# evalf/nutils

Hardware: AMD Instinct MI355X
Metric: elements assembled/sec (global stiffness K) (higher is better)
Workload: dtype f64; 1 GPU; 3D Poisson stiffness, 128^3 structured hex, p=1, 2x2x2 Gauss, iso geometry (BASELINE.json configs[1]); nelems_per_gpu=2097152, nnz_per_gpu=57066625, kernel=k_p1hex_skew<16,16,false,false>, parallelism=single GPU, launch=hipGraph replay (20 steps per graph), settle_steps=600

## Files before the change

nutils_amd/csrc/nh_assemble_p1hex.hip:

```cpp
#include "nh_common.h"
#include <algorithm>
#include <type_traits>
#include <cstdio>
#include <cstdlib>

namespace {

#ifdef NH_ABLATION
#define DEBUG(p) ((p).debug)
#else
#define DEBUG(p) 0
#endif

struct P1Args {
  int n0, n1, n2;
  int lay0, lay1;
  int pl0, pl1;
  const double *verts;
  double origin[3], scale[3];
  double n[2][2];
  double c[3][2];
  double wk[2][2][2];
  double wm[2][2][2];
  int hasm;
// ... 268 lines not shown
          if (kact && (flag & need) == need) {
            const bool below = !upper && dI < 0;
            const double *src0 = acc + (below ? slot_of(Pb - 1) : slot_of(Pb)) + srow, *src1 = acc + (below ? slot_of(Pb) : slot_of(Pb + 1)) + srow;
            double v0[OJ], v1[OJ];
#pragma unroll
            for (int oj = 0; oj < OJ; ++oj) v0[oj] = src0[oj * (VK * NS)];
#pragma unroll
            for (int oj = 0; oj < OJ; ++oj) v1[oj] = src1[oj * (VK * NS)];
            char *lp0 = reinterpret_cast<char *>(p.values + ((3 * (i64)Pb - 1) * T1 * T2 + 3 * (cumJ0 * T2)));
            char *lp1 = lp0 + 8 * (3 * T1 * T2);
#pragma unroll
            for (int oj = 0; oj < OJ; ++oj) {
              *reinterpret_cast<double *>(lp0 + voff8) = v0[oj];
              lp0 += stride8;
            }
#pragma unroll
            for (int oj = 0; oj < OJ; ++oj) {
              *reinterpret_cast<double *>(lp1 + voff8) = v1[oj];
              lp1 += stride8;
            }
          }
        } else if (!lowJ && !highJ) planes(std::integral_constant<int, 0>{});
        else if (!(lowJ && highJ)) planes(std::integral_constant<int, 1>{});
        else planes(std::integral_constant<int, 2>{});
      }
    }
    NH_TICK(4)
    if (last) break;
    lds_barrier();
    NH_TICK(5)
    if (fresh) {
      for (int t = tid; t < NP * PS / 2; t += NT) reinterpret_cast<double2 *>(acc)[t] = make_double2(0., 0.);
    } else {
#pragma unroll
      for (int P = L0 - 1; P < L0 + L - 1; ++P) {
        double2 *z = reinterpret_cast<double2 *>(acc + slot_of(P));
        for (int t = tid; t < PS / 2; t += NT) z[t] = make_double2(0., 0.);
      }
    }
    col = ncol, A = nA, B = nB, L0 = nL0;
    NH_TICK(6)
  }
#ifdef NH_ABLATION
  if (p.tdbg && (tid & 63) == 0)
    for (int i = 0; i < 8; ++i) atomicAdd((unsigned long long *)p.tdbg + i, (unsigned long long)tacc[i]);
#endif
}
#undef NH_TICK

__device__ __forceinline__ void half_arrive(unsigned *cnt) {
  asm volatile("s_waitcnt lgkmcnt(0)" ::: "memory");
  if ((threadIdx.x & 63) == 0) atomicAdd(cnt, 1u);
}
__device__ __forceinline__ void half_wait(unsigned *cnt, unsigned target) {
  while (__hip_atomic_load(cnt, __ATOMIC_RELAXED, __HIP_MEMORY_SCOPE_WORKGROUP) < target) __builtin_amdgcn_s_sleep(1);
  asm volatile("" ::: "memory");
}

#ifdef NH_P1HEX_WPE
#define NH_WPE __attribute__((amdgpu_waves_per_eu(2, 2)))
#else
#define NH_WPE
#endif
template <int TJ, int TK, bool MASS, bool COEF>
__global__ __launch_bounds__(2 * TJ * TK) NH_WPE void k_p1hex_skew(P1Args p) {
  constexpr bool VEC = false;
#ifdef NH_ABLATION
  long long tacc[10] = {0, 0, 0, 0, 0, 0, 0, 0, 0, 0}, tprev = clock64();
  const long long tstart = tprev;
  int nslow = 0, nfast = 0;
#ifdef NH_NOTICKS
#define NH_TICK(i)
#else
#define NH_TICK(i) { const long long tnow = clock64(); tacc[i] += tnow - tprev; tprev = tnow; }
#endif
#else
#define NH_TICK(i)
#endif
  constexpr int G = TJ * TK, NT = 2 * G, NP = 4, OJ = TJ - 1, OK = TK - 1, NS = 15, VW = 3;
  constexpr int VJ = TJ + 1, VK = TK + 1, RP = VJ * VK, PS = (RP * NS + 1) & ~1, VPG = (RP + G - 1) / G;
  const bool getenv_stage_late = p.wbnd < 0;
  extern __shared__ __attribute__((aligned(16))) double lds[];
  double *acc = lds;
  double *vbuf = lds + NP * PS;
  unsigned *hcnt = reinterpret_cast<unsigned *>(vbuf + 3 * RP * VW);
  const int tid = threadIdx.x, lt = tid & (G - 1), grp = __builtin_amdgcn_readfirstlane(tid / G);
  const int N0 = p.n0 + 1, N1 = p.n1 + 1, N2 = p.n2 + 1;
  const int NPL = p.pl1 - p.pl0;
  const unsigned wg = gridDim.x % 8 == 0 ? (blockIdx.x % 8) * (gridDim.x / 8) + blockIdx.x / 8 : blockIdx.x;
  const i64 CP = NPL + 2, WI = 16, WB = p.nbj > 1 ? (p.wbnd < 0 ? -p.wbnd : p.wbnd) : 16;
  const i64 rowB = p.nbk * CP * WB, rowI = p.nbk * CP * WI, nmid = max(p.nbj - 2, 0);
  const i64 ctot = (p.nbj > 1 ? 2 : 1) * rowB + nmid * rowI;
  auto unit_at = [&](i64 c) {
    i64 jt, rem, w;
    if (c < rowB) jt = 0, rem = c, w = WB;
    else if (c < rowB + nmid * rowI) jt = 1 + (c - rowB) / rowI, rem = (c - rowB) % rowI, w = WI;
    else jt = p.nbj > 1 ? p.nbj - 1 : 1, rem = c - rowB - nmid * rowI, w = WB;
    const i64 kt = rem / (CP * w), pos = (rem - kt * CP * w) / w;
    return (jt * p.nbk + kt) * NPL + min(max(pos - 1, (i64)0), (i64)NPL);
  };
  i64 u = unit_at(ctot * wg / gridDim.x);
  const i64 u1 = unit_at(ctot * (wg + 1) / gridDim.x);
  if (u >= u1) return;
  auto slot_of = [](int P) { return (int)((unsigned)(P + 2 * NP) % NP) * PS; };
  auto vslot_of = [](int P) { return (int)((unsigned)(P + 3) % 3) * (RP * VW); };
  auto load_vertex = [&](int I, int r, int J0, int K0, double (&x)[3]) {
    const int bb = r / VK, c = r % VK, J = J0 - 1 + bb, K = K0 - 1 + c;
    x[0] = x[1] = x[2] = 0.;
    if (r < RP && I >= 0 && I < N0 && J >= 0 && J < N1 && K >= 0 && K < N2) {
      const double *src = p.verts + (((i64)I * N1 + J) * N2 + K) * 3;
      x[0] = src[0], x[1] = src[1], x[2] = src[2];
    }
  };
  if (tid == 0) *hcnt = 0;
  unsigned htarget = 0;
  const i64 T1 = 3 * (i64)N1 - 2, T2 = 3 * (i64)N2 - 2;
  while (u < u1) {
    const int col = (int)(u / NPL), A = p.pl0 + (int)(u % NPL), B = (int)min((i64)p.pl1, A + (u1 - u));
    const int J0 = (col / p.nbk) * OJ, K0 = (col % p.nbk) * OK;
    {
      constexpr int NVL = (2 * RP + NT - 1) / NT;
      double x[NVL][3];
      bool valid[NVL];
#pragma unroll
      for (int k = 0; k < NVL; ++k) {
        const int v = min(tid + k * NT, 2 * RP - 1), pl = v / RP, r = v % RP, I = A - 1 + pl;
        const int J = J0 - 1 + r / VK, K = K0 - 1 + r % VK;
        valid[k] = I >= 0 && I < N0 && J >= 0 && J < N1 && K >= 0 && K < N2;
        const double *src = p.verts + (((i64)min(max(I, 0), N0 - 1) * N1 + min(max(J, 0), N1 - 1)) * N2 + min(max(K, 0), N2 - 1)) * 3;
        x[k][0] = src[0], x[k][1] = src[1], x[k][2] = src[2];
      }
      for (int t = tid; t < NP * PS / 2; t += NT) reinterpret_cast<double2 *>(acc)[t] = make_double2(0., 0.);
#pragma unroll
      for (int k = 0; k < NVL; ++k) {
        const int v = tid + k * NT, pl = v / RP, r = v % RP;
        if (v < 2 * RP) {
          double *dst = vbuf + vslot_of(A - 1 + pl) + r * VW;
          dst[0] = valid[k] ? x[k][0] : 0., dst[1] = valid[k] ? x[k][1] : 0., dst[2] = valid[k] ? x[k][2] : 0.;
        }
      }
    }
    lds_barrier();

    for (int s = A - 1; s <= B; ++s) {
      htarget += G / 64;
      NH_TICK(0)
      const bool mathrole = ((s - (A - 1)) & 1) == grp;
#ifdef NH_P1HEX_PRIO
      if (mathrole == (NH_P1HEX_PRIO == 1)) __builtin_amdgcn_s_setprio(3); else __builtin_amdgcn_s_setprio(0);
#endif
      if (mathrole) {
        const int ej = lt / TK, ek = lt % TK;
        const int gi = s, gj = J0 - 1 + ej, gk = K0 - 1 + ek;
        if (s < B && gi >= p.lay0 && gi < p.lay1 && gj >= 0 && gj < p.n1 && gk >= 0 && gk < p.n2 && !(DEBUG(p) & 4)) {
#define NH_P1HEX_VERT(a, bb, c) (vbuf + vslot_of(gi + (a)) + ((ej + (bb)) * VK + (ek + (c))) * VW)
#include "nh_p1hex_element.inc"
#undef NH_P1HEX_VERT
        }
        NH_TICK(3)
      } else {
        const bool needv = s + 1 < B && !(DEBUG(p) & 8);
        double Vn[VPG][3];
#pragma unroll
        for (int k = 0; k < VPG; ++k) load_vertex(needv ? s + 2 : -1, lt + k * G, J0, K0, Vn[k]);
        const int P = s - 1;
        bool arrived = false, staged = false, recycled = false;
        auto stage_vertices = [&]() {
#pragma unroll
          for (int k = 0; k < VPG; ++k) {
            const int r = lt + k * G;
            if (r < RP) {
              double *dst = vbuf + vslot_of(s + 2) + r * VW;
              dst[0] = Vn[k][0], dst[1] = Vn[k][1], dst[2] = Vn[k][2];
            }
          }
        };
        if (P >= A && !(DEBUG(p) & 2)) {
          const bool lowJ = J0 == 0, highJ = J0 + OJ >= N1;
          const int cumJ0 = J0 == 0 ? 0 : 3 * J0 - 1;
#ifdef NH_ABLATION
          if (!lowJ && !highJ && P > 0 && P < N0 - 1 && K0 > 0 && K0 + OK < N2) ++nfast; else ++nslow;
#endif
          if (!lowJ && !highJ && P > 0 && P < N0 - 1 && K0 > 0 && K0 + OK < N2) {
            const int e = 2 * lt;
            auto source = [&](int ee, bool &below) {
              const int ok_ = ee / 27, sl_ = ee - ok_ * 27;
              const int dJ_ = (sl_ / 3) % 3 - 1, dK_ = sl_ % 3 - 1;
              below = sl_ < 9;
              return (VK + ok_ + 1) * NS + (sl_ >= 13 ? sl_ - 13 : (dJ_ * VK + dK_) * NS + 13 - sl_);
            };
#ifdef NH_P1HEX_PIPEFLUSH
            constexpr int D = NH_P1HEX_PIPEFLUSH;
            const int ec = 2 * min(lt, 201);
            bool belowA, belowB;
            const int offA = source(ec, belowA), offB = source(ec + 1, belowB);
            const double *sA = acc + (belowA ? slot_of(P - 1) : slot_of(P)) + offA;
            const double *sB = acc + (belowB ? slot_of(P - 1) : slot_of(P)) + offB;
            const int li = lt - 202;
            const bool lone = li >= 0 && li < OJ;
            bool belowL;
            const int offL = source(404, belowL);
            const double aL = acc[(belowL ? slot_of(P - 1) : slot_of(P)) + offL + (lone ? li : 0) * (VK * NS)];
            const i64 stride8 = 8 * (i64)(9 * (int)T2);
            char *l0 = reinterpret_cast<char *>(p.values + ((3 * (i64)P - 1) * T1 * T2 + 3 * (cumJ0 * T2) + 9 * (3 * (i64)K0 - 1)));
            char *lp = l0 + 8 * ec;
            double a0[OJ], a1[OJ];
#pragma unroll
            for (int i = 0; i < D && i < OJ; ++i) a0[i] = sA[i * (VK * NS)], a1[i] = sB[i * (VK * NS)];
            __builtin_amdgcn_sched_barrier(0);
#pragma unroll
            for (int i = 0; i < OJ; ++i) {
              if (i + D < OJ) a0[i + D] = sA[(i + D) * (VK * NS)], a1[i + D] = sB[(i + D) * (VK * NS)];
              __builtin_amdgcn_sched_barrier(0);
              const double2 v = make_double2(a0[i], a1[i]);
              __builtin_memcpy(lp + i * stride8, &v, 16);
              __builtin_amdgcn_sched_barrier(0);
            }
            half_arrive(hcnt);
            arrived = true;
            if (needv) {
              stage_vertices();
              staged = true;
            }
            __builtin_amdgcn_sched_barrier(0);
            if (lone) *reinterpret_cast<double *>(l0 + li * stride8 + 8 * 404) = aL;
#else
            bool belowA, belowB;
            const int offA = source(e < 405 ? e : 404, belowA), offB = source(e + 1 < 405 ? e + 1 : 404, belowB);
            const double *sA = acc + (belowA ? slot_of(P - 1) : slot_of(P)) + offA;
            const double *sB = acc + (belowB ? slot_of(P - 1) : slot_of(P)) + offB;
            double a0[OJ], a1[OJ];
#pragma unroll
            for (int i = 0; i < OJ; ++i) {
              a0[i] = sA[i * (VK * NS)];
              a1[i] = sB[i * (VK * NS)];
            }
            const int li = lt - 202;
            const bool lone = li >= 0 && li < OJ;
            bool belowL;
            const int offL = source(404, belowL);
            const double aL = acc[(belowL ? slot_of(P - 1) : slot_of(P)) + offL + (lone ? li : 0) * (VK * NS)];
            half_arrive(hcnt);
            arrived = true;
            NH_TICK(8)
            if (needv && !getenv_stage_late) {
              __builtin_amdgcn_s_waitcnt(0x0f70);
              stage_vertices();
              staged = true;
            }
            const i64 stride8 = 8 * (i64)(9 * (int)T2);
            char *l0 = reinterpret_cast<char *>(p.values + ((3 * (i64)P - 1) * T1 * T2 + 3 * (cumJ0 * T2) + 9 * (3 * (i64)K0 - 1)));
            char *lp = l0 + 16 * lt;
#ifdef NH_P1HEX_INTERLEAVE
            half_wait(hcnt, htarget);
            recycled = true;
            {
              double2 *z = reinterpret_cast<double2 *>(acc + slot_of(s - 2));
              constexpr int NZ = (PS / 2 + G - 1) / G;
              static_assert(NZ <= OJ, "one zeroing write per store");
#pragma unroll
              for (int i = 0; i < OJ; ++i) {
                if (lt < 202) {
                  const double2 v = make_double2(a0[i], a1[i]);
                  __builtin_memcpy(lp + i * stride8, &v, 16);
                }
                if (i < NZ && lt + i * G < PS / 2) z[lt + i * G] = make_double2(0., 0.);
                __builtin_amdgcn_sched_barrier(0);
              }
            }
#else
            if (lt < 202) {
#pragma unroll
              for (int i = 0; i < OJ; ++i) {
                if ((DEBUG(p) & 16) && (i & 1)) continue;
                const double2 v = make_double2(a0[i], a1[i]);
                __builtin_memcpy(lp + i * stride8, &v, 16);
              }
            }
#endif
            if (lone) *reinterpret_cast<double *>(l0 + li * stride8 + 8 * 404) = aL;
#endif
          } else {
            constexpr int RPP = G / 32, KP = (OK + RPP - 1) / RPP;
            const int sl = lt & 31, rsub = lt >> 5;
            const int dI = sl / 9 - 1, dJ = (sl / 3) % 3 - 1, dK = sl % 3 - 1;
            const bool upper = sl >= 13;
            const int need = (dI < 0 ? 1 : dI > 0 ? 8 : 0) | (dJ < 0 ? 2 : dJ > 0 ? 16 : 0) | (dK < 0 ? 4 : dK > 0 ? 32 : 0);
            const int loI = P > 0, hiI = P < N0 - 1, lenI = loI + 1 + hiI;
            double v[KP][OJ];
#pragma unroll
            for (int kp = 0; kp < KP; ++kp) {
              const int ok = kp * RPP + rsub;
              const int srow = (VK + ok + 1) * NS + (upper ? sl - 13 : (dJ * VK + dK) * NS + 13 - sl);
              const double *src = acc + ((!upper && dI < 0) ? slot_of(P - 1) : slot_of(P)) + (ok < OK ? srow : 0);
#pragma unroll
              for (int oj = 0; oj < OJ; ++oj) v[kp][oj] = src[oj * (VK * NS)];
            }
            half_arrive(hcnt);
            arrived = true;
#pragma unroll
            for (int kp = 0; kp < KP; ++kp) {
              const int ok = kp * RPP + rsub, Kk = K0 + ok;
              const bool kact = sl < 27 && ok < OK && Kk < N2;
              const int loK = Kk > 0, hiK = Kk < N2 - 1, lenK = loK + 1 + hiK, cumK = Kk == 0 ? 0 : 3 * Kk - 1;
              double *line = p.values + ((P == 0 ? 0 : 3 * (i64)P - 1) * T1 * T2 + lenI * (cumJ0 * T2));
              if (!lowJ && !highJ) {
                const int flag = loI | 2 | loK << 2 | hiI << 3 | 16 | hiK << 5;
                const unsigned voff8 = 8u * (unsigned)(lenI * 3 * cumK + ((dI + loI) * 3 + (dJ + 1)) * lenK + (dK + loK));
                const i64 stride8 = 8 * (i64)(lenI * 3 * (int)T2);
                if (kact && (flag & need) == need) {
                  char *lp = reinterpret_cast<char *>(line);
#pragma unroll
                  for (int oj = 0; oj < OJ; ++oj) {
                    if (!((DEBUG(p) & 16) && (oj & 1))) *reinterpret_cast<double *>(lp + voff8) = v[kp][oj];
                    lp += stride8;
                  }
                }
              } else {
#pragma unroll
                for (int oj = 0; oj < OJ; ++oj) {
                  const int J = J0 + oj;
                  const int loJ = J > 0, hiJ = J < N1 - 1, lenJ = loJ + 1 + hiJ;
                  const int flag = loI | loJ << 1 | loK << 2 | hiI << 3 | hiJ << 4 | hiK << 5;
                  const unsigned voff = (unsigned)(lenI * lenJ * cumK + ((dI + loI) * lenJ + (dJ + loJ)) * lenK + (dK + loK));
                  if (kact && J < N1 && (flag & need) == need && !((DEBUG(p) & 16) && (oj & 1))) line[voff] = v[kp][oj];
                  line += lenI * lenJ * (int)T2;
                }
              }
            }
          }
        }
        NH_TICK(6)
        if (!arrived) half_arrive(hcnt);
        if (!recycled) half_wait(hcnt, htarget);
        NH_TICK(7)
        if (!recycled) {
          double2 *z = reinterpret_cast<double2 *>(acc + slot_of(s - 2));
          for (int t = lt; t < PS / 2; t += G) z[t] = make_double2(0., 0.);
        }
        NH_TICK(9)
        if (needv && !staged) stage_vertices();
      }
      if (mathrole) { NH_TICK(1) } else { NH_TICK(4) }
      lds_barrier();
      if (mathrole) { NH_TICK(2) } else { NH_TICK(5) }
    }
    u += B - A;
  }
#ifdef NH_ABLATION
  if (p.tdbg && tid == 0) {
    p.tdbg[16 + 4 * blockIdx.x] = clock64() - tstart;
    p.tdbg[16 + 4 * blockIdx.x + 1] = nfast;
    p.tdbg[16 + 4 * blockIdx.x + 2] = nslow;
  }
  if (p.tdbg && (tid & 63) == 0)
    for (int i = 0; i < 10; ++i) atomicAdd((unsigned long long *)p.tdbg + i, (unsigned long long)tacc[i]);
#endif
}
#undef NH_TICK

#include "nh_p1hex_tiles.inc"
#include "nh_p1hex_tri.inc"

__global__ void k_p1hex_unit_matrix(P1Args p, double *Ke) {
  double X[2][2][2][3];
  for (int a = 0; a < 2; ++a)
    for (int b = 0; b < 2; ++b)
      for (int c = 0; c < 2; ++c) {
        X[a][b][c][0] = p.origin[0] + p.scale[0] * a;
        X[a][b][c][1] = p.origin[1] + p.scale[1] * b;
        X[a][b][c][2] = p.origin[2] + p.scale[2] * c;
      }
  ElemTables T;
  {
    double (&R0)[3][3] = T.R0, (&R1)[3][3] = T.R1, (&R2)[3][3] = T.R2;
    double (&W01)[2][2][3] = T.W01, (&W02)[2][2][3] = T.W02, (&W12)[2][2][3] = T.W12;
    double (&Mm)[3][3][3] = T.Mm;
    for (int i = 0; i < 27; ++i) (&Mm[0][0][0])[i] = 0.;
    const bool hasm = p.hasm;
#define NH_P1HEX_QS(q) 1.
#define NH_P1HEX_QM(q) 1.
#include "nh_p1hex_math.inc"
#undef NH_P1HEX_QS
#undef NH_P1HEX_QM
  }
#pragma unroll
  for (int a = 0; a < 8; ++a)
#pragma unroll
    for (int b = 0; b < 8; ++b) Ke[a * 8 + b] = element_entry(T, a < b ? a : b, a < b ? b : a);
}

__global__ __launch_bounds__(256) void k_p1hex_uniform(P1Args p, const double *KeG) {
  __shared__ double Ke[64], tabI[2 * 27], tabF[18], tabL[18];
  if (threadIdx.x < 64) Ke[threadIdx.x] = KeG[threadIdx.x];
  __syncthreads();
  const int N0 = p.n0 + 1, N1 = p.n1 + 1, N2 = p.n2 + 1;
  const int I = p.pl0 + blockIdx.x / N1, J = blockIdx.x % N1;
  const i64 T1 = 3 * (i64)N1 - 2, T2 = 3 * (i64)N2 - 2;
// ... 61 lines not shown
  const int slot = (int)(t % 27);
  if (row > row1 || (row == row1 && slot != 0)) return;
  const i64 T1 = 3 * (i64)N1 - 2, T2 = 3 * (i64)N2 - 2;
  auto rp = [&](i64 r) -> i64 {
    if (r >= (i64)N0 * N1 * N2) return (3 * (i64)N0 - 2) * T1 * T2;
    const int Kk = (int)(r % N2), J = (int)((r / N2) % N1), I = (int)(r / ((i64)N2 * N1));
    return cum_of(I, N0) * T1 * T2 + len_of(I, N0) * (cum_of(J, N1) * T2 + (i64)len_of(J, N1) * cum_of(Kk, N2));
  };
  const i64 base = rp(row0);
  if (slot == 0) rowptr[row - row0] = rp(row) - base;
  if (row >= row1) return;
  const int Kk = (int)(row % N2), J = (int)((row / N2) % N1), I = (int)(row / ((i64)N2 * N1));
  const int dI = slot / 9 - 1, dJ = (slot / 3) % 3 - 1, dK = slot % 3 - 1;
  const int cI = I + dI, cJ = J + dJ, cK = Kk + dK;
  if (cI < 0 || cI >= N0 || cJ < 0 || cJ >= N1 || cK < 0 || cK >= N2) return;
  const int lenJ = len_of(J, N1), lenK = len_of(Kk, N2);
  const int pos = ((dI + (I > 0)) * lenJ + (dJ + (J > 0))) * lenK + (dK + (Kk > 0));
  colidx[rp(row) - base + pos] = ((i64)cI * N1 + cJ) * N2 + cK;
}

}

template <bool VEC, bool MASS, bool COEF>
static int launch_march_inst(const nh_p1hex_args *a, P1Args &p, void *stream) {
#ifdef NH_ABLATION
  p.debug = getenv("NH_P1HEX_DEBUG") ? atoi(getenv("NH_P1HEX_DEBUG")) : 0;
#endif
  static const int wbnd_env = getenv("NH_P1HEX_WBND") ? std::min(64, std::max(8, atoi(getenv("NH_P1HEX_WBND")))) : 20;
  p.wbnd = getenv("NH_P1HEX_STAGE_LATE") ? -wbnd_env : wbnd_env;
  constexpr int TJ = 16, TK = 16, L = 2, NTM = L * TJ * TK, NS = VEC ? 1 : 15, VW = VEC ? 4 : 3;
  int dev = 0;
  NH_CHECK_HIP(hipGetDevice(&dev));
  NH_REQUIRE(dev >= 0 && dev < 16, "nh_p1hex: device index %d not supported", dev);
  static int cus_of[16] = {0};
  if (!cus_of[dev]) {
    int n = 256;
    NH_CHECK_HIP(hipDeviceGetAttribute(&n, hipDeviceAttributeMultiprocessorCount, dev));
    cus_of[dev] = n;
  }
  const int cus = cus_of[dev];
  p.nbj = (p.n1 + 1 + TJ - 2) / (TJ - 1);
  p.nbk = (p.n2 + 1 + TK - 2) / (TK - 1);
  const size_t ldsm = sizeof(double) * ((L + 2) * (((TJ + 1) * (TK + 1) * NS + 1) & ~1) + (L + 1) * (TJ + 1) * (TK + 1) * VW + 2);
  const i64 units = (i64)p.nbj * p.nbk * (p.pl1 - p.pl0);
  NH_REQUIRE(a->max_workgroups >= 0, "nh_p1hex: negative max_workgroups");
  unsigned grid = (unsigned)std::min<i64>(units, a->max_workgroups ? std::min(cus, a->max_workgroups) : cus);
#ifdef NH_ABLATION
  if (getenv("NH_P1HEX_MAXWG")) grid = std::min<unsigned>(grid, (unsigned)atoi(getenv("NH_P1HEX_MAXWG")));
#endif
  auto kern = k_p1hex_march<TJ, TK, L, VEC, MASS, COEF>;
  if constexpr (!VEC && L == 2) {
    const char *env = getenv("NH_P1HEX_MARCH"), *kenv = getenv("NH_P1HEX_KERNEL");
    const bool march = (env && atoi(env)) || (kenv && !strcmp(kenv, "march"));
    if (!march) kern = k_p1hex_skew<TJ, TK, MASS, COEF>;
  }
  static const void *attr_set[16][2] = {{nullptr, nullptr}};
  if (attr_set[dev][0] != (const void *)kern && attr_set[dev][1] != (const void *)kern) {
    NH_CHECK_HIP(hipFuncSetAttribute((const void *)kern, hipFuncAttributeMaxDynamicSharedMemorySize, (int)ldsm));
    attr_set[dev][attr_set[dev][0] ? 1 : 0] = (const void *)kern;
  }
#ifdef NH_ABLATION
  static long long *tdbg = nullptr;
  if (!tdbg) NH_CHECK_HIP(hipMalloc((void **)&tdbg, (16 + 4 * 1024) * sizeof(long long)));
  NH_CHECK_HIP(hipMemsetAsync(tdbg, 0, (16 + 4 * 1024) * sizeof(long long), nh_stream(stream)));
  p.tdbg = getenv("NH_P1HEX_TIMERS") ? tdbg : nullptr;
#endif
  hipLaunchKernelGGL(kern, dim3(grid), dim3(NTM), ldsm, nh_stream(stream), p);
  NH_LAUNCH_CHECK();
#ifdef NH_ABLATION
  if (p.tdbg) {
    static long long h[16 + 4 * 1024];
    NH_CHECK_HIP(hipMemcpy(h, tdbg, sizeof h, hipMemcpyDeviceToHost));
    if (getenv("NH_P1HEX_WGTIMES"))
      for (unsigned g = 0; g < grid; ++g) fprintf(stderr, "wg %u cycles %lld fast %lld slow %lld\n", g, h[16 + 4 * g], h[16 + 4 * g + 1], h[16 + 4 * g + 2]);
    const double nw = (double)grid * (NTM / 64);
    if (kern != (void (*)(P1Args))k_p1hex_march<TJ, TK, L, VEC, MASS, COEF>)
      fprintf(stderr, "p1hex_skew cycles per wave: prologue %.0f | math %.0f | - %.0f | math wait %.0f | lds reads %.0f | store issue %.0f | half wait %.0f | zero %.0f | stage %.0f | mem wait %.0f\n", h[0] / nw, h[3] / nw, h[1] / nw,
              h[2] / nw, h[8] / nw, h[6] / nw, h[7] / nw, h[9] / nw, h[4] / nw, h[5] / nw);
    else
    fprintf(stderr, "p1hex_march cycles per wave: stage+next %.0f | B1 %.0f | load+math %.0f | B2 %.0f | stage+flush %.0f | B3 %.0f | zero %.0f\n", h[0] / nw, h[1] / nw,
            h[2] / nw, h[3] / nw, h[4] / nw, h[5] / nw, h[6] / nw);
  }
#endif
  return NH_OK;
}


namespace {
struct TileScratch {
  void *base = nullptr;
  size_t cap = 0;
  unsigned *err_host = nullptr, *err_dev = nullptr;
};
TileScratch g_tiles[16];
}

int nh_p1hex_tiles_release(void) {
  for (auto &t : g_tiles) {
    if (t.base) NH_CHECK_HIP(hipFree(t.base));
    t.base = nullptr, t.cap = 0;
  }
  return NH_OK;
}

template <bool MASS, bool COEF>
static int launch_tiles_inst(const nh_p1hex_args *a, P1Args &p, void *stream) {
  using namespace p1t;
// ... 252 lines not shown
```

nutils_amd/csrc/nh_p1hex_apply.inc:

```
{
  const double (&n)[2][2] = p.n;
  double J0[2][2][3], J1[2][2][3], J2[2][2][3], g0[2][2], g1[2][2], g2[2][2];
#pragma unroll
  for (int d = 0; d < 4; ++d) {
    double e0[2][2], e1[2][2], e2[2][2];
#pragma unroll
    for (int x = 0; x < 2; ++x)
#pragma unroll
      for (int y = 0; y < 2; ++y) {
        if (d < 3) {
          e0[x][y] = X[1][x][y][d < 3 ? d : 0] - X[0][x][y][d < 3 ? d : 0];
          e1[x][y] = X[x][1][y][d < 3 ? d : 0] - X[x][0][y][d < 3 ? d : 0];
          e2[x][y] = X[x][y][1][d < 3 ? d : 0] - X[x][y][0][d < 3 ? d : 0];
        } else {
          e0[x][y] = un[4 + x * 2 + y] - un[x * 2 + y];
          e1[x][y] = un[x * 4 + 2 + y] - un[x * 4 + y];
          e2[x][y] = un[x * 4 + y * 2 + 1] - un[x * 4 + y * 2];
        }
      }
#pragma unroll
    for (int q1 = 0; q1 < 2; ++q1) {
      double t0[2], t1[2], t2[2];
#pragma unroll
      for (int y = 0; y < 2; ++y) {
        t0[y] = n[0][q1] * e0[0][y] + n[1][q1] * e0[1][y];
        t1[y] = n[0][q1] * e1[0][y] + n[1][q1] * e1[1][y];
        t2[y] = n[0][q1] * e2[0][y] + n[1][q1] * e2[1][y];
      }
#pragma unroll
      for (int q2 = 0; q2 < 2; ++q2) {
        const double v0 = n[0][q2] * t0[0] + n[1][q2] * t0[1], v1 = n[0][q2] * t1[0] + n[1][q2] * t1[1], v2 = n[0][q2] * t2[0] + n[1][q2] * t2[1];
        if (d < 3) {
          J0[q1][q2][d < 3 ? d : 0] = v0;
          J1[q1][q2][d < 3 ? d : 0] = v1;
          J2[q1][q2][d < 3 ? d : 0] = v2;
        } else {
          g0[q1][q2] = v0;
          g1[q1][q2] = v1;
          g2[q1][q2] = v2;
        }
      }
    }
  }
  double uq[2][2][2];
  if (hasm) {
    double ua[2][2][2], ub[2][2][2];
#pragma unroll
    for (int x = 0; x < 2; ++x)
#pragma unroll
      for (int y = 0; y < 2; ++y)
#pragma unroll
        for (int qc = 0; qc < 2; ++qc) ua[x][y][qc] = n[0][qc] * un[x * 4 + y * 2] + n[1][qc] * un[x * 4 + y * 2 + 1];
#pragma unroll
    for (int x = 0; x < 2; ++x)
// ... 98 lines not shown
```

nutils_amd/csrc/nh_p1hex_math.inc:

```
{
  const double (&n)[2][2] = p.n;
  const double (&c)[3][2] = p.c;
  double J0[2][2][3], J1[2][2][3], J2[2][2][3];
#pragma unroll
  for (int d = 0; d < 3; ++d) {
    double e0[2][2], e1[2][2], e2[2][2];
#pragma unroll
    for (int x = 0; x < 2; ++x)
#pragma unroll
      for (int y = 0; y < 2; ++y) {
        e0[x][y] = X[1][x][y][d] - X[0][x][y][d];
        e1[x][y] = X[x][1][y][d] - X[x][0][y][d];
        e2[x][y] = X[x][y][1][d] - X[x][y][0][d];
      }
    double t0[2][2], t1[2][2], t2[2][2];
#pragma unroll
    for (int y = 0; y < 2; ++y) {
      const double d0 = e0[1][y] - e0[0][y], d1 = e1[1][y] - e1[0][y], d2 = e2[1][y] - e2[0][y];
#pragma unroll
      for (int q1 = 0; q1 < 2; ++q1) {
        t0[q1][y] = fma(n[1][q1], d0, e0[0][y]);
        t1[q1][y] = fma(n[1][q1], d1, e1[0][y]);
        t2[q1][y] = fma(n[1][q1], d2, e2[0][y]);
      }
    }
#pragma unroll
    for (int q1 = 0; q1 < 2; ++q1) {
      const double d0 = t0[q1][1] - t0[q1][0], d1 = t1[q1][1] - t1[q1][0], d2 = t2[q1][1] - t2[q1][0];
#pragma unroll
      for (int q2 = 0; q2 < 2; ++q2) {
        J0[q1][q2][d] = fma(n[1][q2], d0, t0[q1][0]);
        J1[q1][q2][d] = fma(n[1][q2], d1, t1[q1][0]);
        J2[q1][q2][d] = fma(n[1][q2], d2, t2[q1][0]);
      }
    }
  }
  double D0[2][2], D1[2][2], D2[2][2], M01[2][2][2], M02[2][2][2], M12[2][2][2], Dm[2][2][2];
#pragma unroll
  for (int qa = 0; qa < 2; ++qa)
#pragma unroll
    for (int qb = 0; qb < 2; ++qb)
#pragma unroll
      for (int qc = 0; qc < 2; ++qc) {
        const double *c0 = J0[qb][qc], *c1 = J1[qa][qc], *c2 = J2[qa][qb];
        double A[3][3];
        A[0][0] = c1[1] * c2[2] - c1[2] * c2[1];
        A[0][1] = c1[2] * c2[0] - c1[0] * c2[2];
        A[0][2] = c1[0] * c2[1] - c1[1] * c2[0];
        A[1][0] = c2[1] * c0[2] - c2[2] * c0[1];
        A[1][1] = c2[2] * c0[0] - c2[0] * c0[2];
        A[1][2] = c2[0] * c0[1] - c2[1] * c0[0];
        A[2][0] = c0[1] * c1[2] - c0[2] * c1[1];
        A[2][1] = c0[2] * c1[0] - c0[0] * c1[2];
        A[2][2] = c0[0] * c1[1] - c0[1] * c1[0];
        const double det = c0[0] * A[0][0] + c0[1] * A[0][1] + c0[2] * A[0][2];
// ... 130 lines not shown
```

Baseline: 12.29 billion elements/s.

## Cut address arithmetic and register pressure in skewed p1hex assembly kernel

Reworks the skewed-wavefront hex assembly loop to carry rotating ring indices, vertex slot offsets and the global output line pointer incrementally instead of recomputing modulo and 64-bit index math each plane. The state moves to 32-bit unsigned scheduling values made uniform via readfirstlane, and kernel arguments are read through a scalar kernarg pointer. Per-lane LDS source offsets are hoisted out of the loop, and the scatter reads use inline-asm ds_read_b64 with immediate offsets. Other changes: a single-lane wave arrive via exec masking, a boundary-lane mask hoisted per column, and unrolled slot zeroing. It adds a host-side limit check for 32-bit overflow and removes the pipeflush/interleave variants.

Measured after the change: 12.25 billion elements/s. About the same (-0.3%).

```diff
diff --git a/nutils_amd/csrc/nh_assemble_p1hex.hip b/nutils_amd/csrc/nh_assemble_p1hex.hip
--- a/nutils_amd/csrc/nh_assemble_p1hex.hip
+++ b/nutils_amd/csrc/nh_assemble_p1hex.hip
@@ -344,6 +344,11 @@
   asm volatile("s_waitcnt lgkmcnt(0)" ::: "memory");
   if ((threadIdx.x & 63) == 0) atomicAdd(cnt, 1u);
 }
+__device__ __forceinline__ void half_arrive_wave(unsigned *cnt) {
+  unsigned long long saved;
+  asm volatile("s_waitcnt lgkmcnt(0)\n\ts_mov_b64 %0, exec\n\ts_mov_b64 exec, 1\n\tds_add_u32 %1, %2\n\ts_mov_b64 exec, %0"
+               : "=&s"(saved) : "v"((unsigned)(size_t)cnt), "v"(1u) : "memory");
+}
 __device__ __forceinline__ void half_wait(unsigned *cnt, unsigned target) {
   while (__hip_atomic_load(cnt, __ATOMIC_RELAXED, __HIP_MEMORY_SCOPE_WORKGROUP) < target) __builtin_amdgcn_s_sleep(1);
   asm volatile("" ::: "memory");
@@ -354,6 +359,32 @@
 #else
 #define NH_WPE
 #endif
+__device__ __forceinline__ int uni(int x) { return __builtin_amdgcn_readfirstlane(x); }
+__device__ __forceinline__ unsigned lane_offset(unsigned x) {
+  asm volatile("" : "+v"(x));
+  return x;
+}
+typedef double double2v __attribute__((ext_vector_type(2)));
+template <int OFF>
+__device__ __forceinline__ double lds_rd64(unsigned a) {
+  static_assert(OFF >= 0 && OFF < 65536, "offset field of a DS instruction");
+  double v;
+  asm volatile("ds_read_b64 %0, %1 offset:%2" : "=v"(v) : "v"(a), "n"(OFF));
+  return v;
+}
+template <int N, int STRIDE, int I = 0>
+__device__ __forceinline__ void lds_rd64_pairs(unsigned a, unsigned b, double2v (&v)[N]) {
+  if constexpr (I < N) {
+    v[I].x = lds_rd64<I * STRIDE>(a);
+    v[I].y = lds_rd64<I * STRIDE>(b);
+    lds_rd64_pairs<N, STRIDE, I + 1>(a, b, v);
+  }
+}
+__device__ __forceinline__ void lds_tie(double2v &x) { asm volatile("" : "+v"(x)); }
+__device__ __forceinline__ int scalar_here(int x) {
+  asm volatile("" : "+s"(x));
+  return x;
+}
 template <int TJ, int TK, bool MASS, bool COEF>
 __global__ __launch_bounds__(2 * TJ * TK) NH_WPE void k_p1hex_skew(P1Args p) {
   constexpr bool VEC = false;
@@ -371,45 +402,56 @@
 #endif
   constexpr int G = TJ * TK, NT = 2 * G, NP = 4, OJ = TJ - 1, OK = TK - 1, NS = 15, VW = 3;
   constexpr int VJ = TJ + 1, VK = TK + 1, RP = VJ * VK, PS = (RP * NS + 1) & ~1, VPG = (RP + G - 1) / G;
+  static_assert((NP & (NP - 1)) == 0 && G % 64 == 0, "ring of plane slots: a power of two; whole waves per half");
   const bool getenv_stage_late = p.wbnd < 0;
   extern __shared__ __attribute__((aligned(16))) double lds[];
   double *acc = lds;
   double *vbuf = lds + NP * PS;
   unsigned *hcnt = reinterpret_cast<unsigned *>(vbuf + 3 * RP * VW);
-  const int tid = threadIdx.x, lt = tid & (G - 1), grp = __builtin_amdgcn_readfirstlane(tid / G);
+  const int tid = threadIdx.x, lt = tid & (G - 1), grp = uni(tid / G), wv = uni(lt >> 6);
   const int N0 = p.n0 + 1, N1 = p.n1 + 1, N2 = p.n2 + 1;
   const int NPL = p.pl1 - p.pl0;
   const unsigned wg = gridDim.x % 8 == 0 ? (blockIdx.x % 8) * (gridDim.x / 8) + blockIdx.x / 8 : blockIdx.x;
-  const i64 CP = NPL + 2, WI = 16, WB = p.nbj > 1 ? (p.wbnd < 0 ? -p.wbnd : p.wbnd) : 16;
-  const i64 rowB = p.nbk * CP * WB, rowI = p.nbk * CP * WI, nmid = max(p.nbj - 2, 0);
-  const i64 ctot = (p.nbj > 1 ? 2 : 1) * rowB + nmid * rowI;
-  auto unit_at = [&](i64 c) {
-    i64 jt, rem, w;
+  const unsigned CP = NPL + 2, WI = 16, WB = p.nbj > 1 ? (unsigned)(p.wbnd < 0 ? -p.wbnd : p.wbnd) : 16u;
+  const unsigned rowB = p.nbk * CP * WB, rowI = p.nbk * CP * WI, nmid = max(p.nbj - 2, 0);
+  const unsigned ctot = (p.nbj > 1 ? 2 : 1) * rowB + nmid * rowI;
+  auto unit_at = [&](unsigned c) {
+    unsigned jt, rem, w;
     if (c < rowB) jt = 0, rem = c, w = WB;
     else if (c < rowB + nmid * rowI) jt = 1 + (c - rowB) / rowI, rem = (c - rowB) % rowI, w = WI;
     else jt = p.nbj > 1 ? p.nbj - 1 : 1, rem = c - rowB - nmid * rowI, w = WB;
-    const i64 kt = rem / (CP * w), pos = (rem - kt * CP * w) / w;
-    return (jt * p.nbk + kt) * NPL + min(max(pos - 1, (i64)0), (i64)NPL);
+    const unsigned kt = rem / (CP * w), pos = (rem - kt * CP * w) / w;
+    return (jt * p.nbk + kt) * NPL + (pos == 0 ? 0u : min(pos - 1, (unsigned)NPL));
   };
-  i64 u = unit_at(ctot * wg / gridDim.x);
-  const i64 u1 = unit_at(ctot * (wg + 1) / gridDim.x);
+  auto share = [&](unsigned w) { return (ctot / gridDim.x) * w + (ctot % gridDim.x) * w / gridDim.x; };
+  unsigned u = (unsigned)uni((int)unit_at(share(wg)));
+  const unsigned u1 = (unsigned)uni((int)unit_at(share(wg + 1)));
   if (u >= u1) return;
-  auto slot_of = [](int P) { return (int)((unsigned)(P + 2 * NP) % NP) * PS; };
   auto vslot_of = [](int P) { return (int)((unsigned)(P + 3) % 3) * (RP * VW); };
-  auto load_vertex = [&](int I, int r, int J0, int K0, double (&x)[3]) {
-    const int bb = r / VK, c = r % VK, J = J0 - 1 + bb, K = K0 - 1 + c;
-    x[0] = x[1] = x[2] = 0.;
-    if (r < RP && I >= 0 && I < N0 && J >= 0 && J < N1 && K >= 0 && K < N2) {
-      const double *src = p.verts + (((i64)I * N1 + J) * N2 + K) * 3;
-      x[0] = src[0], x[1] = src[1], x[2] = src[2];
-    }
-  };
   if (tid == 0) *hcnt = 0;
   unsigned htarget = 0;
   const i64 T1 = 3 * (i64)N1 - 2, T2 = 3 * (i64)N2 - 2;
+  const i64 pstr = T1 * T2;
+  const i64 vplane = 24 * (i64)N1 * N2;
+  const int ej = lt / TK, ek = lt % TK, erow = (ej * VK + ek) * NS, evert = (ej * VK + ek) * VW;
+  auto source = [&](int ee, int &below) {
+    const int ok_ = ee / 27, sl_ = ee - ok_ * 27;
+    const int dJ_ = (sl_ / 3) % 3 - 1, dK_ = sl_ % 3 - 1;
+    below = sl_ < 9;
+    return 8 * ((VK + ok_ + 1) * NS + (sl_ >= 13 ? sl_ - 13 : (dJ_ * VK + dK_) * NS + 13 - sl_));
+  };
+  const int lp2 = min(lt, 201), li = min(max(lt - 202, 0), OJ - 1);
+  static_assert(202 / 64 == (202 + OJ - 1) / 64, "the lone entries of a pass are stored by one wave");
+  int belowA, belowB, belowL;
+  const int srcA = source(2 * lp2, belowA), srcB = source(2 * lp2 + 1, belowB);
+  const int srcL = source(404, belowL) + li * (VK * NS * 8);
+  belowA = (int)lane_offset(belowA), belowB = (int)lane_offset(belowB);
   while (u < u1) {
-    const int col = (int)(u / NPL), A = p.pl0 + (int)(u % NPL), B = (int)min((i64)p.pl1, A + (u1 - u));
-    const int J0 = (col / p.nbk) * OJ, K0 = (col % p.nbk) * OK;
+    const int col = uni((int)(u / (unsigned)NPL)), A = uni(p.pl0 + (int)(u - (unsigned)col * NPL)), B = uni(min(p.pl1, A + (int)(u1 - u)));
+    const int jt = uni(col / p.nbk), J0 = uni(jt * OJ), K0 = uni((col - jt * p.nbk) * OK);
+    const bool lowJ = J0 == 0, highJ = J0 + OJ >= N1;
+    const bool icol = !lowJ && !highJ && K0 > 0 && K0 + OK < N2;
+    const int cumJ0 = J0 == 0 ? 0 : 3 * J0 - 1;
     {
       constexpr int NVL = (2 * RP + NT - 1) / NT;
       double x[NVL][3];
@@ -432,146 +474,107 @@
         }
       }
     }
+    const bool elane = J0 - 1 + ej >= 0 && J0 - 1 + ej < p.n1 && K0 - 1 + ek >= 0 && K0 - 1 + ek < p.n2;
+    unsigned voff[VPG];
+#pragma unroll
+    for (int k = 0; k < VPG; ++k) {
+      const int r = min(lt + k * G, RP - 1), J = J0 - 1 + r / VK, K = K0 - 1 + r % VK;
+      voff[k] = 24u * (unsigned)(min(max(J, 0), N1 - 1) * N2 + min(max(K, 0), N2 - 1));
+    }
+    int ri = uni((A - 1 + 2 * NP) & (NP - 1));
+    int vs0 = uni(vslot_of(A - 1)), vs1 = uni(vslot_of(A)), vs2 = uni(vslot_of(A + 1));
+    int turn = 0;
+    i64 lineP = 8 * ((3 * (i64)(A - 2) - 1) * pstr + 3 * (cumJ0 * T2) + 9 * (3 * (i64)K0 - 1));
     lds_barrier();
 
     for (int s = A - 1; s <= B; ++s) {
       htarget += G / 64;
       NH_TICK(0)
-      const bool mathrole = ((s - (A - 1)) & 1) == grp;
+      const bool mathrole = turn == grp;
+      const int sl_m2 = ((ri + 2) & (NP - 1)) * PS, sl_m1 = ((ri + 3) & (NP - 1)) * PS, sl_0 = ri * PS, sl_p1 = ((ri + 1) & (NP - 1)) * PS;
 #ifdef NH_P1HEX_PRIO
       if (mathrole == (NH_P1HEX_PRIO == 1)) __builtin_amdgcn_s_setprio(3); else __builtin_amdgcn_s_setprio(0);
 #endif
       if (mathrole) {
-        const int ej = lt / TK, ek = lt % TK;
         const int gi = s, gj = J0 - 1 + ej, gk = K0 - 1 + ek;
-        if (s < B && gi >= p.lay0 && gi < p.lay1 && gj >= 0 && gj < p.n1 && gk >= 0 && gk < p.n2 && !(DEBUG(p) & 4)) {
-#define NH_P1HEX_VERT(a, bb, c) (vbuf + vslot_of(gi + (a)) + ((ej + (bb)) * VK + (ek + (c))) * VW)
+        if (s < B && gi >= p.lay0 && gi < p.lay1 && !(DEBUG(p) & 4)) {
+          unsigned long long ka = reinterpret_cast<unsigned long long>(__builtin_amdgcn_kernarg_segment_ptr());
+          asm volatile("" : "+s"(ka));
+          const __attribute__((address_space(4))) P1Args &p = *reinterpret_cast<const __attribute__((address_space(4))) P1Args *>(ka);
+          if (elane) {
+            double *const plq[2] = {acc + sl_0 + erow, acc + sl_p1 + erow};
+            const double *const vq[2] = {vbuf + vs0 + evert, vbuf + vs1 + evert};
+#define NH_P1HEX_SLOT(a0, a1, a2, b0, b1, b2) (plq[a0] + ((a1) * VK + (a2)) * NS + ((b0) - (a0)) * 9 + ((b1) - (a1)) * 3 + ((b2) - (a2)))
+#define NH_P1HEX_VERT(a, bb, c) (vq[a] + ((bb) * VK + (c)) * VW)
 #include "nh_p1hex_element.inc"
 #undef NH_P1HEX_VERT
+#undef NH_P1HEX_SLOT
+          }
         }
         NH_TICK(3)
       } else {
         const bool needv = s + 1 < B && !(DEBUG(p) & 8);
         double Vn[VPG][3];
-#pragma unroll
-        for (int k = 0; k < VPG; ++k) load_vertex(needv ? s + 2 : -1, lt + k * G, J0, K0, Vn[k]);
+        auto has_nodes = [&](int k) { return (k + 1) * G <= RP || k * G + wv * 64 < RP; };
+#pragma unroll
+        for (int k = 0; k < VPG; ++k) Vn[k][0] = Vn[k][1] = Vn[k][2] = 0.;
+        if (needv) {
+          const char *vpl = reinterpret_cast<const char *>(p.verts) + (i64)min(s + 2, N0 - 1) * vplane;
+#pragma unroll
+          for (int k = 0; k < VPG; ++k) {
+            if (has_nodes(k)) {
+              const double *src = reinterpret_cast<const double *>(vpl + (size_t)lane_offset(voff[k]));
+              Vn[k][0] = src[0], Vn[k][1] = src[1], Vn[k][2] = src[2];
+            }
+          }
+        }
         const int P = s - 1;
-        bool arrived = false, staged = false, recycled = false;
+        bool arrived = false, staged = false;
         auto stage_vertices = [&]() {
 #pragma unroll
           for (int k = 0; k < VPG; ++k) {
-            const int r = lt + k * G;
-            if (r < RP) {
-              double *dst = vbuf + vslot_of(s + 2) + r * VW;
+            const int r = min(lt + k * G, RP - 1);
+            if (has_nodes(k)) {
+              double *dst = vbuf + vs2 + r * VW;
               dst[0] = Vn[k][0], dst[1] = Vn[k][1], dst[2] = Vn[k][2];
             }
           }
         };
         if (P >= A && !(DEBUG(p) & 2)) {
-          const bool lowJ = J0 == 0, highJ = J0 + OJ >= N1;
-          const int cumJ0 = J0 == 0 ? 0 : 3 * J0 - 1;
 #ifdef NH_ABLATION
-          if (!lowJ && !highJ && P > 0 && P < N0 - 1 && K0 > 0 && K0 + OK < N2) ++nfast; else ++nslow;
-#endif
-          if (!lowJ && !highJ && P > 0 && P < N0 - 1 && K0 > 0 && K0 + OK < N2) {
-            const int e = 2 * lt;
-            auto source = [&](int ee, bool &below) {
-              const int ok_ = ee / 27, sl_ = ee - ok_ * 27;
-              const int dJ_ = (sl_ / 3) % 3 - 1, dK_ = sl_ % 3 - 1;
-              below = sl_ < 9;
-              return (VK + ok_ + 1) * NS + (sl_ >= 13 ? sl_ - 13 : (dJ_ * VK + dK_) * NS + 13 - sl_);
-            };
-#ifdef NH_P1HEX_PIPEFLUSH
-            constexpr int D = NH_P1HEX_PIPEFLUSH;
-            const int ec = 2 * min(lt, 201);
-            bool belowA, belowB;
-            const int offA = source(ec, belowA), offB = source(ec + 1, belowB);
-            const double *sA = acc + (belowA ? slot_of(P - 1) : slot_of(P)) + offA;
-            const double *sB = acc + (belowB ? slot_of(P - 1) : slot_of(P)) + offB;
-            const int li = lt - 202;
-            const bool lone = li >= 0 && li < OJ;
-            bool belowL;
-            const int offL = source(404, belowL);
-            const double aL = acc[(belowL ? slot_of(P - 1) : slot_of(P)) + offL + (lone ? li : 0) * (VK * NS)];
-            const i64 stride8 = 8 * (i64)(9 * (int)T2);
-            char *l0 = reinterpret_cast<char *>(p.values + ((3 * (i64)P - 1) * T1 * T2 + 3 * (cumJ0 * T2) + 9 * (3 * (i64)K0 - 1)));
-            char *lp = l0 + 8 * ec;
-            double a0[OJ], a1[OJ];
-#pragma unroll
-            for (int i = 0; i < D && i < OJ; ++i) a0[i] = sA[i * (VK * NS)], a1[i] = sB[i * (VK * NS)];
-            __builtin_amdgcn_sched_barrier(0);
-#pragma unroll
-            for (int i = 0; i < OJ; ++i) {
-              if (i + D < OJ) a0[i + D] = sA[(i + D) * (VK * NS)], a1[i + D] = sB[(i + D) * (VK * NS)];
-              __builtin_amdgcn_sched_barrier(0);
-              const double2 v = make_double2(a0[i], a1[i]);
-              __builtin_memcpy(lp + i * stride8, &v, 16);
-              __builtin_amdgcn_sched_barrier(0);
-            }
-            half_arrive(hcnt);
+          if (icol && P > 0 && P < N0 - 1) ++nfast; else ++nslow;
+#endif
+          if (icol && P > 0 && P < N0 - 1) {
+            const char *const accb = reinterpret_cast<const char *>(acc);
+            const int dbelow = 8 * (sl_m2 - sl_m1);
+            const unsigned accP = (unsigned)(size_t)acc + 8u * (unsigned)sl_m1;
+            double2v a01[OJ];
+            lds_rd64_pairs<OJ, VK * NS * 8>(accP + (unsigned)(srcA + __mul24(belowA, dbelow)), accP + (unsigned)(srcB + __mul24(belowB, dbelow)), a01);
+            const double aL = *reinterpret_cast<const double *>(accb + (8 * sl_m1 + srcL));
+            half_arrive_wave(hcnt);
             arrived = true;
-            if (needv) {
-              stage_vertices();
-              staged = true;
-            }
-            __builtin_amdgcn_sched_barrier(0);
-            if (lone) *reinterpret_cast<double *>(l0 + li * stride8 + 8 * 404) = aL;
-#else
-            bool belowA, belowB;
-            const int offA = source(e < 405 ? e : 404, belowA), offB = source(e + 1 < 405 ? e + 1 : 404, belowB);
-            const double *sA = acc + (belowA ? slot_of(P - 1) : slot_of(P)) + offA;
-            const double *sB = acc + (belowB ? slot_of(P - 1) : slot_of(P)) + offB;
-            double a0[OJ], a1[OJ];
-#pragma unroll
-            for (int i = 0; i < OJ; ++i) {
-              a0[i] = sA[i * (VK * NS)];
-              a1[i] = sB[i * (VK * NS)];
-            }
-            const int li = lt - 202;
-            const bool lone = li >= 0 && li < OJ;
-            bool belowL;
-            const int offL = source(404, belowL);
-            const double aL = acc[(belowL ? slot_of(P - 1) : slot_of(P)) + offL + (lone ? li : 0) * (VK * NS)];
-            half_arrive(hcnt);
-            arrived = true;
+#pragma unroll
+            for (int i = 0; i < OJ; ++i) lds_tie(a01[i]);
             NH_TICK(8)
             if (needv && !getenv_stage_late) {
               __builtin_amdgcn_s_waitcnt(0x0f70);
               stage_vertices();
               staged = true;
             }
-            const i64 stride8 = 8 * (i64)(9 * (int)T2);
-            char *l0 = reinterpret_cast<char *>(p.values + ((3 * (i64)P - 1) * T1 * T2 + 3 * (cumJ0 * T2) + 9 * (3 * (i64)K0 - 1)));
-            char *lp = l0 + 16 * lt;
-#ifdef NH_P1HEX_INTERLEAVE
-            half_wait(hcnt, htarget);
-            recycled = true;
+            const i64 stride8 = 8 * (9 * T2);
+            char *const l0 = reinterpret_cast<char *>(p.values) + lineP;
+            const unsigned lane16 = lane_offset(16u * (unsigned)lp2);
             {
-              double2 *z = reinterpret_cast<double2 *>(acc + slot_of(s - 2));
-              constexpr int NZ = (PS / 2 + G - 1) / G;
-              static_assert(NZ <= OJ, "one zeroing write per store");
+              char *lp = l0;
 #pragma unroll
               for (int i = 0; i < OJ; ++i) {
-                if (lt < 202) {
-                  const double2 v = make_double2(a0[i], a1[i]);
-                  __builtin_memcpy(lp + i * stride8, &v, 16);
+                if (!((DEBUG(p) & 16) && (i & 1))) {
+                  __builtin_memcpy(lp + (size_t)lane16, &a01[i], 16);
                 }
-                if (i < NZ && lt + i * G < PS / 2) z[lt + i * G] = make_double2(0., 0.);
-                __builtin_amdgcn_sched_barrier(0);
+                lp += stride8;
               }
             }
-#else
-            if (lt < 202) {
-#pragma unroll
-              for (int i = 0; i < OJ; ++i) {
-                if ((DEBUG(p) & 16) && (i & 1)) continue;
-                const double2 v = make_double2(a0[i], a1[i]);
-                __builtin_memcpy(lp + i * stride8, &v, 16);
-              }
-            }
-#endif
-            if (lone) *reinterpret_cast<double *>(l0 + li * stride8 + 8 * 404) = aL;
-#endif
+            if (wv == 202 / 64) *reinterpret_cast<double *>(l0 + (size_t)lane_offset((unsigned)li * (unsigned)stride8 + 8u * 404u)) = aL;
           } else {
             constexpr int RPP = G / 32, KP = (OK + RPP - 1) / RPP;
             const int sl = lt & 31, rsub = lt >> 5;
@@ -584,18 +587,18 @@
             for (int kp = 0; kp < KP; ++kp) {
               const int ok = kp * RPP + rsub;
               const int srow = (VK + ok + 1) * NS + (upper ? sl - 13 : (dJ * VK + dK) * NS + 13 - sl);
-              const double *src = acc + ((!upper && dI < 0) ? slot_of(P - 1) : slot_of(P)) + (ok < OK ? srow : 0);
+              const double *src = acc + ((!upper && dI < 0) ? sl_m2 : sl_m1) + (ok < OK ? srow : 0);
 #pragma unroll
               for (int oj = 0; oj < OJ; ++oj) v[kp][oj] = src[oj * (VK * NS)];
             }
-            half_arrive(hcnt);
+            half_arrive_wave(hcnt);
             arrived = true;
 #pragma unroll
             for (int kp = 0; kp < KP; ++kp) {
               const int ok = kp * RPP + rsub, Kk = K0 + ok;
               const bool kact = sl < 27 && ok < OK && Kk < N2;
               const int loK = Kk > 0, hiK = Kk < N2 - 1, lenK = loK + 1 + hiK, cumK = Kk == 0 ? 0 : 3 * Kk - 1;
-              double *line = p.values + ((P == 0 ? 0 : 3 * (i64)P - 1) * T1 * T2 + lenI * (cumJ0 * T2));
+              double *line = p.values + ((P == 0 ? 0 : 3 * (i64)P - 1) * pstr + lenI * (cumJ0 * T2));
               if (!lowJ && !highJ) {
                 const int flag = loI | 2 | loK << 2 | hiI << 3 | 16 | hiK << 5;
                 const unsigned voff8 = 8u * (unsigned)(lenI * 3 * cumK + ((dI + loI) * 3 + (dJ + 1)) * lenK + (dK + loK));
@@ -609,9 +612,10 @@
                   }
                 }
               } else {
+                const int J0h = scalar_here(J0);
 #pragma unroll
                 for (int oj = 0; oj < OJ; ++oj) {
-                  const int J = J0 + oj;
+                  const int J = J0h + oj;
                   const int loJ = J > 0, hiJ = J < N1 - 1, lenJ = loJ + 1 + hiJ;
                   const int flag = loI | loJ << 1 | loK << 2 | hiI << 3 | hiJ << 4 | hiK << 5;
                   const unsigned voff = (unsigned)(lenI * lenJ * cumK + ((dI + loI) * lenJ + (dJ + loJ)) * lenK + (dK + loK));
@@ -623,12 +627,16 @@
           }
         }
         NH_TICK(6)
-        if (!arrived) half_arrive(hcnt);
-        if (!recycled) half_wait(hcnt, htarget);
+        if (!arrived) half_arrive_wave(hcnt);
+        half_wait(hcnt, htarget);
         NH_TICK(7)
-        if (!recycled) {
-          double2 *z = reinterpret_cast<double2 *>(acc + slot_of(s - 2));
-          for (int t = lt; t < PS / 2; t += G) z[t] = make_double2(0., 0.);
+        {
+          double2 *z = reinterpret_cast<double2 *>(acc + sl_m2) + lt;
+          constexpr int NZ = PS / 2 / G;
+          static_assert(PS / 2 >= G, "a plane slot is at least one pass");
+#pragma unroll
+          for (int k = 0; k < NZ; ++k) z[k * G] = make_double2(0., 0.);
+          if (PS / 2 % G) z[PS / 2 - G] = make_double2(0., 0.);
         }
         NH_TICK(9)
         if (needv && !staged) stage_vertices();
@@ -636,6 +644,10 @@
       if (mathrole) { NH_TICK(1) } else { NH_TICK(4) }
       lds_barrier();
       if (mathrole) { NH_TICK(2) } else { NH_TICK(5) }
+      ri = (ri + 1) & (NP - 1);
+      { const int t = vs0; vs0 = vs1, vs1 = vs2, vs2 = t; }
+      turn ^= 1;
+      lineP += 24 * pstr;
     }
     u += B - A;
   }
@@ -803,7 +815,12 @@
   if constexpr (!VEC && L == 2) {
     const char *env = getenv("NH_P1HEX_MARCH"), *kenv = getenv("NH_P1HEX_KERNEL");
     const bool march = (env && atoi(env)) || (kenv && !strcmp(kenv, "march"));
-    if (!march) kern = k_p1hex_skew<TJ, TK, MASS, COEF>;
+    if (!march) {
+      kern = k_p1hex_skew<TJ, TK, MASS, COEF>;
+      const i64 N1 = p.n1 + 1, N2 = p.n2 + 1;
+      NH_REQUIRE((i64)p.nbj * p.nbk * (p.pl1 - p.pl0 + 2) * 64 < ((i64)1 << 31) && 24 * N1 * N2 < ((i64)1 << 32) && TJ * 72 * (3 * N2 - 2) < ((i64)1 << 32),
+                 "nh_p1hex: mesh too large for the 32-bit run state of the skewed kernel (NH_P1HEX_KERNEL=march has no such limit)");
+    }
   }
   static const void *attr_set[16][2] = {{nullptr, nullptr}};
   if (attr_set[dev][0] != (const void *)kern && attr_set[dev][1] != (const void *)kern) {
diff --git a/nutils_amd/csrc/nh_p1hex_apply.inc b/nutils_amd/csrc/nh_p1hex_apply.inc
--- a/nutils_amd/csrc/nh_p1hex_apply.inc
+++ b/nutils_amd/csrc/nh_p1hex_apply.inc
@@ -1,5 +1,5 @@
 {
-  const double (&n)[2][2] = p.n;
+  const auto &n = p.n;
   double J0[2][2][3], J1[2][2][3], J2[2][2][3], g0[2][2], g1[2][2], g2[2][2];
 #pragma unroll
   for (int d = 0; d < 4; ++d) {
diff --git a/nutils_amd/csrc/nh_p1hex_math.inc b/nutils_amd/csrc/nh_p1hex_math.inc
--- a/nutils_amd/csrc/nh_p1hex_math.inc
+++ b/nutils_amd/csrc/nh_p1hex_math.inc
@@ -1,6 +1,6 @@
 {
-  const double (&n)[2][2] = p.n;
-  const double (&c)[3][2] = p.c;
+  const auto &n = p.n;
+  const auto &c = p.c;
   double J0[2][2][3], J1[2][2][3], J2[2][2][3];
 #pragma unroll
   for (int d = 0; d < 3; ++d) {
```
